# shiyao-li/NextBestPath

Measured on AMD Instinct MI355X. Metric: exploration steps/s (+ NBP maps/s) at 256x256, higher is better.
Workload: dtype f32

## Files before the change

nextbestpath_amd/csrc/nbp_conv.hip:

```cpp
#include "common.h"
#include "nbp_internal.h"
#include "nbp_first_conv.h"
#include <cstdlib>



template <int WM, int WN, int TM, int TN>
__global__ __launch_bounds__(256, 2) void igemm_conv_kernel(IgemmArgs a) {
    int zs = blockIdx.z;
    if (zs >= a.split_k) {
        zs -= a.split_k;
        a.src0 = a.g_src0; a.src1 = a.g_src1; a.wpk = a.g_wpk; a.scale = a.g_scale; a.shift = a.g_shift; a.out = a.g_out;
    }
    constexpr int BM = WM * TM * 32, BN = WN * TN * 32;
    constexpr int RA = BM / 32, RB = BN / 32;
    constexpr int STAGE = (BM + BN) * 32;
    static_assert(WM * WN == 4, "256-thread workgroup");
    extern __shared__ __attribute__((aligned(16))) float lds[];
    const int tid = threadIdx.x, lane = tid & 63, wave = tid >> 6;
    const int wm = wave / WN, wn = wave % WN;
    unsigned mt = blockIdx.x, nt = blockIdx.y;
    if (a.xcd_remap) {
        const unsigned L = blockIdx.x + gridDim.x * blockIdx.y, T = gridDim.x * gridDim.y;
        const unsigned xcd = L & 7u, idx = L >> 3, q = T >> 3, r = T & 7u;
// ... 638 lines not shown

__global__ __launch_bounds__(256) void conv_first_mfma_linear_kernel(const float* __restrict__ x, int B, int H, int W,
                                                                     const float* __restrict__ w, const float* __restrict__ scale,
                                                                     const float* __restrict__ shift, float* __restrict__ out) {
    auto st4 = [](float* p, const f32x4& v) { *reinterpret_cast<f32x4*>(p) = v; };
    conv_first_mfma_body<float, decltype(st4), false>(x, B, H, W, w, scale, shift, out, st4, nullptr);
}

static unsigned first_grid(long long M) {
    constexpr int cap = 512;
    const long long tiles = M / 256;
    return (unsigned)(tiles < cap ? tiles : cap);
}

int nbp_conv_first_amax_launch(const float* x_nchw, int B, int H, int W, const float* w_oihw, const float* scale, const float* shift,
                               float* out_nhwc, unsigned* amax_out, int* did_amax, hipStream_t st) {
    long long M = (long long)B * H * W;
    *did_amax = 0;
    if ((H & 7) == 0 && (W & 31) == 0) {
        conv_first_mfma_kernel<<<first_grid(M), 256, 0, st>>>(x_nchw, B, H, W, w_oihw, scale, shift, out_nhwc, amax_out);
        *did_amax = amax_out ? 1 : 0;
        return nbp_launch_status();
    }
    return nbp_conv_first_f32(x_nchw, B, H, W, w_oihw, scale, shift, out_nhwc, st);
}

extern "C" int nbp_conv_first_f32(const float* x_nchw, int B, int H, int W, const float* w_oihw, const float* scale,
                                  const float* shift, float* out_nhwc, void* stream) {
    NBP_ENTER();
    NBP_RETURN_IF(!x_nchw || !w_oihw || !scale || !shift || !out_nhwc, NBP_E_ARG);
    NBP_RETURN_IF(B < 1 || H < 1 || W < 1, NBP_E_ARG);
    long long M = (long long)B * H * W;
    if ((H & 7) == 0 && (W & 31) == 0) {
        conv_first_mfma_kernel<<<first_grid(M), 256, 0, (hipStream_t)stream>>>(x_nchw, B, H, W, w_oihw, scale, shift, out_nhwc, nullptr);
        return nbp_launch_status();
    }
    conv_first_kernel<<<(unsigned)nbp_cdiv(M, 64), 256, 0, (hipStream_t)stream>>>(x_nchw, B, H, W, w_oihw, scale,
                                                                                   shift, out_nhwc);
    return nbp_launch_status();
}

extern "C" int nbp_conv_first_linear_f32(const float* x_nchw, int B, int H, int W, const float* w_oihw, const float* scale,
                                         const float* shift, float* out_nhwc, void* stream) {
    NBP_ENTER();
    NBP_RETURN_IF(!x_nchw || !w_oihw || !scale || !shift || !out_nhwc || B < 1, NBP_E_ARG);
    NBP_RETURN_IF(H < 8 || W < 32 || (H & 7) || (W & 31), NBP_E_SHAPE);
    conv_first_mfma_linear_kernel<<<first_grid((long long)B * H * W), 256, 0, (hipStream_t)stream>>>(x_nchw, B, H, W, w_oihw, scale, shift, out_nhwc);
    return nbp_launch_status();
}

__global__ __launch_bounds__(256) void maxpool2_kernel(const float* __restrict__ in, int B, int H, int W, int C4,
                                                       float* __restrict__ out) {
    const int Ho = H >> 1, Wo = W >> 1;
    const long long total = (long long)B * Ho * Wo * C4;
    const f32x4* in4 = reinterpret_cast<const f32x4*>(in);
    f32x4* out4 = reinterpret_cast<f32x4*>(out);
    for (long long i = (long long)blockIdx.x * blockDim.x + threadIdx.x; i < total;
         i += (long long)gridDim.x * blockDim.x) {
        int c = (int)(i % C4);
        long long p = i / C4;
        int xo = (int)(p % Wo);
        long long q = p / Wo;
        int yo = (int)(q % Ho);
        int b = (int)(q / Ho);
        long long base = (((long long)b * H + 2 * yo) * W + 2 * xo) * C4 + c;
        f32x4 v0 = in4[base], v1 = in4[base + C4], v2 = in4[base + (long long)W * C4],
              v3 = in4[base + (long long)W * C4 + C4];
        f32x4 r;
#pragma unroll
        for (int e = 0; e < 4; ++e) r[e] = fmaxf(fmaxf(v0[e], v1[e]), fmaxf(v2[e], v3[e]));
        out4[i] = r;
    }
}

extern "C" int nbp_maxpool2_nhwc_f32(const float* in, int B, int H, int W, int C, float* out, void* stream) {
    NBP_ENTER();
    NBP_RETURN_IF(!in || !out, NBP_E_ARG);
    NBP_RETURN_IF(B < 1 || H < 2 || W < 2 || (H & 1) || (W & 1) || C < 4 || (C & 3), NBP_E_SHAPE);
    long long total = (long long)B * (H / 2) * (W / 2) * (C / 4);
    maxpool2_kernel<<<nbp_ew_grid(total, 256), 256, 0, (hipStream_t)stream>>>(in, B, H, W, C / 4, out);
    return nbp_launch_status();
}

__global__ __launch_bounds__(256) void psi_gate_kernel(const float* __restrict__ q, int F4,
                                                       const float* __restrict__ wpsi, const float* __restrict__ st,
                                                       const float* __restrict__ x, int C4, long long M,
                                                       float* __restrict__ out) {
    const int sub = threadIdx.x & 15;
    const f32x4* q4 = reinterpret_cast<const f32x4*>(q);
    const f32x4* w4 = reinterpret_cast<const f32x4*>(wpsi);
    const f32x4* x4 = reinterpret_cast<const f32x4*>(x);
    f32x4* o4 = reinterpret_cast<f32x4*>(out);
    const float s = st[0], t = st[1];
    const long long ppb = blockDim.x >> 4;
    for (long long m = (long long)blockIdx.x * ppb + (threadIdx.x >> 4); m < M; m += (long long)gridDim.x * ppb) {
        float acc = 0.f;
        for (int f = sub; f < F4; f += 16) {
            f32x4 a = q4[m * F4 + f], b = w4[f];
            acc = fmaf(a[0], b[0], acc); acc = fmaf(a[1], b[1], acc);
            acc = fmaf(a[2], b[2], acc); acc = fmaf(a[3], b[3], acc);
        }
        acc += __shfl_xor(acc, 8, 16);
        acc += __shfl_xor(acc, 4, 16);
        acc += __shfl_xor(acc, 2, 16);
        acc += __shfl_xor(acc, 1, 16);
        const float z = acc * s + t;
        const float psi = 1.f / (1.f + expf(-z));
        for (int c = sub; c < C4; c += 16) o4[m * C4 + c] = x4[m * C4 + c] * psi;
    }
}

extern "C" int nbp_psi_gate_f32(const float* q, int F, const float* w_psi, const float* s_t2, const float* x, int C,
                                long long M, float* out, void* stream) {
    NBP_ENTER();
    NBP_RETURN_IF(!q || !w_psi || !s_t2 || !x || !out, NBP_E_ARG);
    NBP_RETURN_IF(F < 4 || (F & 3) || C < 4 || (C & 3) || M < 1, NBP_E_SHAPE);
    psi_gate_kernel<<<nbp_ew_grid(M * 16, 256), 256, 0, (hipStream_t)stream>>>(q, F / 4, w_psi, s_t2, x, C / 4, M,
                                                                                out);
    return nbp_launch_status();
}

template <int NO>
__global__ __launch_bounds__(256) void final_1x1_kernel(const float* __restrict__ in, int B, int H, int W, int C4,
                                                        const float* __restrict__ w, const float* __restrict__ scale,
                                                        const float* __restrict__ shift, int sigmoid,
                                                        float* __restrict__ out) {
    const int sub = threadIdx.x & 15;
    const f32x4* in4 = reinterpret_cast<const f32x4*>(in);
    const f32x4* w4 = reinterpret_cast<const f32x4*>(w);
    const long long HW = (long long)H * W, M = (long long)B * HW;
    const long long ppb = blockDim.x >> 4;
    for (long long m = (long long)blockIdx.x * ppb + (threadIdx.x >> 4); m < M; m += (long long)gridDim.x * ppb) {
        float acc[NO];
#pragma unroll
        for (int o = 0; o < NO; ++o) acc[o] = 0.f;
        for (int c = sub; c < C4; c += 16) {
            f32x4 v = in4[m * C4 + c];
#pragma unroll
            for (int o = 0; o < NO; ++o) {
                f32x4 ww = w4[o * C4 + c];
                acc[o] = fmaf(v[0], ww[0], acc[o]); acc[o] = fmaf(v[1], ww[1], acc[o]);
                acc[o] = fmaf(v[2], ww[2], acc[o]); acc[o] = fmaf(v[3], ww[3], acc[o]);
            }
        }
#pragma unroll
        for (int o = 0; o < NO; ++o) {
            acc[o] += __shfl_xor(acc[o], 8, 16);
            acc[o] += __shfl_xor(acc[o], 4, 16);
            acc[o] += __shfl_xor(acc[o], 2, 16);
            acc[o] += __shfl_xor(acc[o], 1, 16);
        }
        if (sub == 0) {
            const long long b = m / HW, rem = m - b * HW;
#pragma unroll
            for (int o = 0; o < NO; ++o) {
                float v = acc[o] * scale[o] + shift[o];
                if (sigmoid) v = 1.f / (1.f + expf(-v));
                out[(b * NO + o) * HW + rem] = v;
            }
        }
    }
}

extern "C" int nbp_final_1x1_f32(const float* in, int B, int H, int W, int C, const float* w_oc, int n_out,
                                 const float* scale, const float* shift, int sigmoid, float* out_nchw, void* stream) {
    NBP_ENTER();
    NBP_RETURN_IF(!in || !w_oc || !scale || !shift || !out_nchw, NBP_E_ARG);
    NBP_RETURN_IF(B < 1 || H < 1 || W < 1 || C < 4 || (C & 3), NBP_E_SHAPE);
    long long M = (long long)B * H * W;
    int grid = nbp_ew_grid(M * 16, 256);
    hipStream_t st = (hipStream_t)stream;
    if (n_out == 8) final_1x1_kernel<8><<<grid, 256, 0, st>>>(in, B, H, W, C / 4, w_oc, scale, shift, sigmoid, out_nchw);
    else if (n_out == 1) final_1x1_kernel<1><<<grid, 256, 0, st>>>(in, B, H, W, C / 4, w_oc, scale, shift, sigmoid, out_nchw);
    else return NBP_E_SHAPE;
    return nbp_launch_status();
}

__global__ void nchw_to_nhwc_kernel(const float* __restrict__ in, int B, int C, long long HW, float* __restrict__ out) {
    const long long total = (long long)B * C * HW;
    for (long long i = (long long)blockIdx.x * blockDim.x + threadIdx.x; i < total;
         i += (long long)gridDim.x * blockDim.x) {
        int c = (int)(i % C);
        long long p = i / C;
        long long b = p / HW, hw = p - b * HW;
        out[i] = in[(b * C + c) * HW + hw];
    }
}
__global__ void nhwc_to_nchw_kernel(const float* __restrict__ in, int B, int C, long long HW, float* __restrict__ out) {
    const long long total = (long long)B * C * HW;
    for (long long i = (long long)blockIdx.x * blockDim.x + threadIdx.x; i < total;
         i += (long long)gridDim.x * blockDim.x) {
        long long hw = i % HW;
        long long p = i / HW;
        int c = (int)(p % C);
        long long b = p / C;
        out[i] = in[(b * HW + hw) * C + c];
    }
}
extern "C" int nbp_nchw_to_nhwc_f32(const float* in, int B, int C, int H, int W, float* out, void* stream) {
    NBP_ENTER();
    NBP_RETURN_IF(!in || !out || B < 1 || C < 1 || H < 1 || W < 1, NBP_E_ARG);
    long long total = (long long)B * C * H * W;
    nchw_to_nhwc_kernel<<<nbp_ew_grid(total, 256), 256, 0, (hipStream_t)stream>>>(in, B, C, (long long)H * W, out);
    return nbp_launch_status();
}
extern "C" int nbp_nhwc_to_nchw_f32(const float* in, int B, int C, int H, int W, float* out, void* stream) {
    NBP_ENTER();
    NBP_RETURN_IF(!in || !out || B < 1 || C < 1 || H < 1 || W < 1, NBP_E_ARG);
    long long total = (long long)B * C * H * W;
    nhwc_to_nchw_kernel<<<nbp_ew_grid(total, 256), 256, 0, (hipStream_t)stream>>>(in, B, C, (long long)H * W, out);
    return nbp_launch_status();
}
```

nextbestpath_amd/csrc/nbp_forward.hip:

```cpp
#include "common.h"
#include "nbp_internal.h"
#include <stdio.h>
#include <stdlib.h>
#include <string.h>

namespace {

enum Kind { K_FIRST, K_CONV3, K_ATT_G, K_ATT_X, K_PSI, K_FINAL };
struct LayerSpec { Kind kind; int cin, cout, k; };

struct Table {
    LayerSpec L[NBP_N_CONV];
    size_t w_off[NBP_N_CONV];
    size_t s_off[NBP_N_CONV], t_off[NBP_N_CONV];
    size_t total_floats;
    size_t w3_off[NBP_N_CONV];
    size_t w3u_off[NBP_N_CONV];
    bool is_up[NBP_N_CONV];
    int up_rank[NBP_N_CONV];
    size_t total3_bytes;
    size_t wup16_off[NBP_N_CONV], total_up16_bytes;
    size_t w1_off[NBP_N_CONV];
    int gate_rank[NBP_N_CONV];
    Table() {
// ... 201 lines not shown
                break;
        }
    }
    if (rc) { free(h); return rc; }
    *handle_out = h;
    return 0;
}

extern "C" int nbp_pack_weights(const void* const* w_host_array, const void* const* scale_host_array,
                                const void* const* shift_host_array, void* packed, size_t packed_bytes, void* stream,
                                nbp_weights** handle_out) {
    NBP_ENTER();
    return pack_weights_impl(w_host_array, scale_host_array, shift_host_array, packed, packed_bytes, stream, handle_out,
                             false);
}

extern "C" int nbp_pack_weights_bf16(const void* const* w_host_array, const void* const* scale_host_array,
                                     const void* const* shift_host_array, void* packed, size_t packed_bytes,
                                     void* stream, nbp_weights** handle_out) {
    NBP_ENTER();
    return pack_weights_impl(w_host_array, scale_host_array, shift_host_array, packed, packed_bytes, stream, handle_out,
                             true);
}

extern "C" size_t nbp_packed_weights_bytes_split(void) { return table().total_floats * sizeof(float) + table().total3_bytes; }
extern "C" int nbp_pack_weights_split(const void* const* w_host_array, const void* const* scale_host_array,
                                      const void* const* shift_host_array, void* packed, size_t packed_bytes,
                                      void* stream, nbp_weights** handle_out) {
    NBP_ENTER();
    return pack_weights_impl(w_host_array, scale_host_array, shift_host_array, packed, packed_bytes, stream, handle_out,
                             false, true);
}

extern "C" size_t nbp_packed_weights_bytes_bf16(void) { return table().total_floats * sizeof(float) + table().total_up16_bytes; }

extern "C" void nbp_free_weights(nbp_weights* handle) { free(handle); }

namespace {

struct Bump {
    char* base; size_t size, off; bool dry;
    template <typename T> T* take(size_t count) {
        size_t bytes = (count * sizeof(T) + 255) / 256 * 256;
        size_t o = off; off += bytes;
        if (dry) return (T*)(uintptr_t)256;
        return (T*)(base + o);
    }
};

struct Timer {
    hipStream_t st;
    nbp_layer_timing* out; int cap; int n;
    hipEvent_t ev[256];
    int nev;
    int begin() {
        nev = 0; n = 0;
        hipError_t e = hipEventCreate(&ev[0]);
        if (e != hipSuccess) return (int)e;
        nev = 1;
        return (int)hipEventRecord(ev[0], st);
    }
    void mark(const char* name, double flops, int tile, int split_k, long long M, int N, int K) {
        if (n >= cap || nev >= 256) return;
        if (hipEventCreate(&ev[nev]) != hipSuccess) return;
        (void)hipEventRecord(ev[nev], st);
        ++nev;
        nbp_layer_timing& t = out[n++];
        memset(&t, 0, sizeof(t));
        strncpy(t.name, name, sizeof(t.name) - 1);
        t.flops = flops; t.tile = tile; t.split_k = split_k; t.M = M; t.N = N; t.K = K;
    }
    int finish() {
        hipError_t e = hipStreamSynchronize(st);
        for (int i = 0; i + 1 < nev && i < n; ++i) {
            float ms = 0.f;
            (void)hipEventElapsedTime(&ms, ev[i], ev[i + 1]);
            out[i].ms = ms;
        }
        for (int i = 0; i < nev; ++i) (void)hipEventDestroy(ev[i]);
        return (int)e;
    }
};

struct NoCtx {
    int init(Bump&, hipStream_t, bool) { return 0; }
    void offer_gated(void*, void*) {}
    bool took_gated() { return false; }
    void offer_pool(void*) {}
    bool took_pool() { return false; }
    void offer_head(const float*, const float*, const float*, float*) {}
    bool took_head() { return false; }
};
struct PathF32 {
    typedef float T;
    typedef ConvOperands Ops;
    typedef NoCtx Ctx;
    static constexpr int CHUNK = 32;
    static ConvPlan plan(long long M, int N, int chunks, int groups, int H = 0, int ksize = 0, int ups = 0) {
        (void)ups;
        return nbp_plan_conv(M, N, chunks, 0, 0, groups, H, H, ksize);
    }
    static constexpr int MODE = 0;
    template <typename C>
    static int conv(C&, const nbp_weights*, const int*, const Ops& o, const Ops* o2, int C0, int C1, int ups, int B, int H, int ks,
                    int N, void* ws, size_t wsb, hipStream_t st) {
        return nbp_conv_igemm_launch_g(o, o2, C0, C1, ups, B, H, H, ks, N, 1, 0, 0, ws, wsb, st);
    }
    template <typename C>
    static int first(C&, const float* x, int B, int s, const nbp_weights* h, T* out, hipStream_t st) {
        return nbp_conv_first_f32(x, B, s, s, (const float*)h->w[0], h->scale[0], h->shift[0], out, st);
    }
    template <typename C>
    static int pool(C&, const T* in, int B, int H, int Cn, T* out, hipStream_t st) { return nbp_maxpool2_nhwc_f32(in, B, H, H, Cn, out, st); }
    template <typename C>
    static int gate(C&, const T* q, int F, const float* w, const float* s2, const T* x, int Cn, long long M, T* out, hipStream_t st) {
        return nbp_psi_gate_f32(q, F, w, s2, x, Cn, M, out, st);
    }
    static int head(const T* in, int B, int H, int C, const float* w, int no, const float* sc, const float* sh, int sig,
                    float* out, hipStream_t st) {
        return nbp_final_1x1_f32(in, B, H, H, C, w, no, sc, sh, sig, out, st);
    }
};
struct AmaxBook {
    unsigned* slots = nullptr;
    int next = 0, n = 0;
    hipStream_t st = nullptr;
    const void* key[128];
    unsigned* val[128];
    int init(Bump& bp, hipStream_t s, bool dry) {
        st = s; next = n = 0;
        slots = bp.take<unsigned>(128 * 64);
        return dry ? 0 : fill_f32(reinterpret_cast<float*>(slots), 0.f, 128 * 64, st);
    }
    unsigned* find(const void* p) const {
        for (int i = n - 1; i >= 0; --i) if (key[i] == p) return val[i];
        return nullptr;
    }
    void bind(const void* p, unsigned* v) { if (n < 128) { key[n] = p; val[n] = v; ++n; } }
    unsigned* unbound() { return next < 128 ? slots + 64 * next++ : nullptr; }
    unsigned* fresh(const void* p) { unsigned* v = next < 128 ? slots + 64 * next++ : nullptr; if (v) bind(p, v); return v; }
    void alias(const void* p, const void* of) { if (unsigned* v = find(of)) bind(p, v); }
    float* gated[2] = {nullptr, nullptr};
    bool gated_taken = false;
    void offer_gated(void* g0, void* g1) { gated[0] = (float*)g0; gated[1] = (float*)g1; gated_taken = false; }
    bool took_gated() { const bool t = gated_taken; gated[0] = gated[1] = nullptr; gated_taken = false; return t; }
    const float* psi_key[2] = {nullptr, nullptr};
    const float* psi_x[2] = {nullptr, nullptr};
    float* pool = nullptr;
    bool pool_taken = false;
    void offer_pool(void* p) { pool = (float*)p; pool_taken = false; }
    bool took_pool() { const bool t = pool_taken; pool = nullptr; pool_taken = false; return t; }
    ConvHead head = {nullptr, nullptr, nullptr, nullptr};
    bool head_taken = false;
    void offer_head(const float* w, const float* sc, const float* sh, float* out) { head = ConvHead{w, sc, sh, out}; head_taken = false; }
    bool took_head() { const bool t = head_taken; head = ConvHead{nullptr, nullptr, nullptr, nullptr}; head_taken = false; return t; }
    int ensure(const float* p, long long count, const unsigned** out) {
        unsigned* v = find(p);
        int rc = 0;
        if (!v) {
            v = fresh(p);
            if (!v) return NBP_E_WS;
            rc = nbp_amax_launch(p, count, v, st);
        }
        *out = v;
        return rc;
    }
};
struct PathSplit : PathF32 {
    typedef AmaxBook Ctx;
    static constexpr int MODE = 2;
    static ConvPlan plan(long long M, int N, int chunks, int groups, int H = 0, int ksize = 0, int ups = 0) {
        if (ksize == 1) return ConvPlan{NBP_TILE_SPLIT_GATE, 1, chunks};
        const ConvPlan p = nbp_plan_conv_split(M, N, chunks, 0, groups, H, H, ksize, ups);
        return p.tile ? p : PathF32::plan(M, N, chunks, groups, H, ksize);
    }
    static int conv(Ctx& ctx, const nbp_weights* h, const int* li, const Ops& o, const Ops* o2, int C0, int C1, int ups, int B,
                    int H, int ks, int N, void* ws, size_t wsb, hipStream_t st) {
        if (ks == 1 && C1 == C0 && C0 % 64 == 0 && !ups && h->w1[li[0]] && (!o2 || h->w1[li[1]])) {
            const long long M = (long long)B * H * H;
            ConvOperandsSplit s[2];
            for (int g = 0; g < (o2 ? 2 : 1); ++g) {
                const Ops& q = g ? *o2 : o;
                s[g] = ConvOperandsSplit{q.src0, q.src1, h->w1[li[g]], q.scale, q.shift, q.out, nullptr, nullptr, h->wamax1[li[g]], nullptr,
                                         nullptr, nullptr};
                int rc = ctx.ensure(q.src0, M * C0, &s[g].amax0);
                if (!rc) rc = ctx.ensure(q.src1, M * C1, &s[g].amax1);
                if (rc) return rc;
            }
            GatePsi psi;
            for (int g = 0; g < 2; ++g) {
                const int l = li[(g && o2) ? 1 : 0] + 2;
                psi.wpsi[g] = (const float*)h->w[l]; psi.st[g] = h->scale[l]; psi.gated[g] = ctx.gated[(g && o2) ? 1 : 0];
            }
            unsigned* gslot[2] = {nullptr, nullptr};
            if (ctx.gated[0]) for (int g = 0; g < (o2 ? 2 : 1); ++g) psi.gated_amax[g] = gslot[g] = ctx.unbound();
            static const int psi_on_load = nbp_tune_int("NBP_SPLIT_PSI_ON_LOAD", 1);
            const ConvPlan pc = nbp_plan_conv_split(M, C0, (C0 + C0) / 32 * 9, 0, o2 ? 2 : 1, H, H, 3, 0);
            psi.psi_only = psi_on_load && (C0 >= 128 || psi_on_load >= 2) && ctx.gated[0] && gslot[0] && (!o2 || gslot[1]) && pc.tile != 0 &&
                           M * C0 * 4 < (1ll << 31);
            int fused = 0;
            const int rc = nbp_gate1x1_split_launch_g(s[0], o2 ? &s[1] : nullptr, C0, M, N, 1, st, ctx.gated[0] ? &psi : nullptr, &fused);
            if (fused) {
                ctx.gated_taken = true;
                for (int g = 0; g < (o2 ? 2 : 1); ++g) {
                    if (gslot[g]) ctx.bind(ctx.gated[g], gslot[g]);
                    else ctx.alias(ctx.gated[g], (g ? *o2 : o).src1);
                    if (psi.psi_only) { ctx.psi_key[g] = ctx.gated[g]; ctx.psi_x[g] = (g ? *o2 : o).src1; }
                }
            }
            return rc;
        }
        const ConvPlan p = nbp_plan_conv_split((long long)B * H * H, N, (C0 + C1) / 32 * ks * ks, 0, o2 ? 2 : 1, H, H, ks, ups);
        if (!p.tile) return PathF32::conv(ctx, h, li, o, o2, C0, C1, ups, B, H, ks, N, ws, wsb, st);
        const long long hw = (long long)B * (ups ? H / 2 : H) * (ups ? H / 2 : H);
        ConvOperandsSplit s[2];
        for (int g = 0; g < (o2 ? 2 : 1); ++g) {
            const Ops& q = g ? *o2 : o;
            s[g] = ConvOperandsSplit{q.src0, q.src1, h->w3[li[g]], q.scale, q.shift, q.out, nullptr, nullptr, h->wamax[li[g]], nullptr,
                                     h->w3u[li[g]], h->wamax_u[li[g]]};
            int rc = ctx.ensure(q.src0, hw * C0, &s[g].amax0);
            if (!rc && C1) rc = ctx.ensure(q.src1, hw * C1, &s[g].amax1);
            if (rc) return rc;
            s[g].amax_out = ctx.fresh(q.out);
            for (int k = 0; k < 2; ++k)
                if (ctx.psi_key[k] && q.src0 == ctx.psi_key[k]) {
                    s[g].src0 = ctx.psi_x[k]; s[g].psi0 = ctx.psi_key[k];
                    ctx.psi_key[k] = nullptr; ctx.psi_x[k] = nullptr;
                }
        }
        float* pools[2] = {ctx.pool, nullptr};
        int pooled = 0, headed = 0;
        const int rc = nbp_conv_split_launch_g(s[0], o2 ? &s[1] : nullptr, C0, C1, ups, B, H, H, ks, N, 1, 0, ws, wsb, st,
                                               (ctx.pool && !o2) ? pools : nullptr, &pooled, (ctx.head.out && !o2) ? &ctx.head : nullptr,
                                               &headed);
        if (headed) ctx.head_taken = true;
        if (pooled) {
            ctx.pool_taken = true;
            ctx.alias(ctx.pool, o.out);
        }
        return rc;
    }
    static int first(Ctx& ctx, const float* x, int B, int s, const nbp_weights* h, T* out, hipStream_t st) {
        unsigned* slot = ctx.fresh(out);
        int did = 0;
        const int rc = nbp_conv_first_amax_launch(x, B, s, s, (const float*)h->w[0], h->scale[0], h->shift[0], out, slot, &did, st);
        if (!did && slot) --ctx.n;
        return rc;
    }
    static int pool(Ctx& ctx, const T* in, int B, int H, int Cn, T* out, hipStream_t st) {
        ctx.alias(out, in);
        return nbp_maxpool2_nhwc_f32(in, B, H, H, Cn, out, st);
    }
    static int gate(Ctx& ctx, const T* q, int F, const float* w, const float* s2, const T* x, int Cn, long long M, T* out,
                    hipStream_t st) {
        ctx.alias(out, x);
        return nbp_psi_gate_f32(q, F, w, s2, x, Cn, M, out, st);
    }
};
struct Bf16Ctx : NoCtx {
    bf16_t* gated[2] = {nullptr, nullptr};
    bool gated_taken = false;
    void offer_gated(void* g0, void* g1) { gated[0] = (bf16_t*)g0; gated[1] = (bf16_t*)g1; gated_taken = false; }
    bool took_gated() { const bool t = gated_taken; gated[0] = gated[1] = nullptr; gated_taken = false; return t; }
    bf16_t* pool = nullptr;
    bool pool_taken = false;
    void offer_pool(void* p) { pool = (bf16_t*)p; pool_taken = false; }
    bool took_pool() { const bool t = pool_taken; pool = nullptr; pool_taken = false; return t; }
    ConvHead head = {nullptr, nullptr, nullptr, nullptr};
    bool head_taken = false;
    void offer_head(const float* w, const float* sc, const float* sh, float* out) { head = ConvHead{w, sc, sh, out}; head_taken = false; }
    bool took_head() { const bool t = head_taken; head = ConvHead{nullptr, nullptr, nullptr, nullptr}; head_taken = false; return t; }
};
struct PathBF16 {
    typedef bf16_t T;
    typedef ConvOperandsH Ops;
    typedef Bf16Ctx Ctx;
    static constexpr int CHUNK = 64;
    static ConvPlan plan(long long M, int N, int chunks, int groups, int H = 0, int ksize = 0, int ups = 0) {
        return nbp_plan_conv_bf16(M, N, chunks, 0, 0, groups, H, H, ksize, ups);
    }
    static constexpr int MODE = 1;
    static int conv(Ctx& ctx, const nbp_weights* h, const int* li, const Ops& o, const Ops* o2, int C0, int C1, int ups, int B, int H,
                    int ks, int N, void* ws, size_t wsb, hipStream_t st) {
        Ops a = o, b = o2 ? *o2 : o;
        a.wpk_up = (const bf16_t*)h->wup16[li[0]];
        if (o2) b.wpk_up = (const bf16_t*)h->wup16[li[1]];
        bf16_t* pools[2] = {ctx.pool, nullptr};
        int pooled = 0, headed = 0, psi_fused = 0;
        GatePsiH psi{{nullptr, nullptr}, {nullptr, nullptr}, {nullptr, nullptr}};
        const bool gate = ks == 1 && C1 == C0 && ctx.gated[0] && (!o2 || ctx.gated[1]);
        if (gate)
            for (int g = 0; g < (o2 ? 2 : 1); ++g) {
                const int l = li[g] + 2;
                psi.wpsi[g] = (const float*)h->w[l]; psi.st[g] = h->scale[l]; psi.gated[g] = ctx.gated[g];
            }
        const int rc = nbp_conv_igemm_bf16_launch_g(a, o2 ? &b : nullptr, C0, C1, ups, B, H, H, ks, N, 1, 0, 0, ws, wsb, st,
                                                    (ctx.pool && !o2) ? pools : nullptr, &pooled,
                                                    (ctx.head.out && !o2) ? &ctx.head : nullptr, &headed, gate ? &psi : nullptr, &psi_fused);
        if (pooled) ctx.pool_taken = true;
        if (headed) ctx.head_taken = true;
        if (psi_fused) ctx.gated_taken = true;
        return rc;
    }
    static int first(Ctx&, const float* x, int B, int s, const nbp_weights* h, T* out, hipStream_t st) {
        return nbp_conv_first_bf16_launch(x, B, s, s, (const float*)h->w[0], h->scale[0], h->shift[0], out, st);
    }
    static int pool(Ctx&, const T* in, int B, int H, int C, T* out, hipStream_t st) { return nbp_maxpool2_bf16_launch(in, B, H, H, C, out, st); }
    static int gate(Ctx&, const T* q, int F, const float* w, const float* s2, const T* x, int C, long long M, T* out, hipStream_t st) {
        return nbp_psi_gate_bf16_launch(q, F, w, s2, x, C, M, out, st);
    }
    static int head(const T* in, int B, int H, int C, const float* w, int no, const float* sc, const float* sh, int sig,
                    float* out, hipStream_t st) {
        return nbp_final_1x1_bf16_launch(in, B, H, H, C, w, no, sc, sh, sig, out, st);
    }
};

template <typename P>
size_t splitk_scratch_floats(long long M, int N, int cin_total, int taps, int groups, int H, int ups = 0) {
    ConvPlan p = P::plan(M, N, cin_total / P::CHUNK * taps, groups, H, taps == 9 ? 3 : 1, ups);
    return p.split_k > 1 ? (size_t)groups * p.split_k * M * N : 0;
}

template <typename P>
int run_forward(const nbp_weights* h, const float* x, int B, int S, float* out1, float* out2, Bump& bp,
                hipStream_t st, Timer* tm = nullptr) {
    typedef typename P::T T;
    typedef typename P::Ops Ops;
    char nm[48];
    const bool dry = bp.dry;
    const int enc[5] = {64, 128, 256, 512, 1024};
    int rc = 0;
    size_t sk = 0;
    {
        int s = S;
        sk = 0;
        for (int e = 0; e < 5; ++e, s /= 2) {
            long long M = (long long)B * s * s;
            if (e > 0) sk = max(sk, splitk_scratch_floats<P>(M, enc[e], enc[e - 1], 9, 1, s));
            sk = max(sk, splitk_scratch_floats<P>(M, enc[e], enc[e], 9, 1, s));
            if (e < 4) {
                for (int g = 1; g <= 2; ++g) {
                    sk = max(sk, splitk_scratch_floats<P>(M, enc[e], enc[e + 1], 9, g, s));
                    sk = max(sk, splitk_scratch_floats<P>(M, enc[e], enc[e + 1], 9, g, s, 1));
                    sk = max(sk, splitk_scratch_floats<P>(M, enc[e], enc[e], 9, g, s));
                    sk = max(sk, splitk_scratch_floats<P>(M, enc[e], 2 * enc[e], 9, g, s));
                    sk = max(sk, splitk_scratch_floats<P>(M, enc[e] / 2, 2 * enc[e], 1, g, s));
                }
            }
        }
    }
    float* skws = bp.take<float>(sk ? sk : 64);
    const size_t skbytes = sk * sizeof(float);
    typename P::Ctx ctx;
    rc = ctx.init(bp, st, dry);

    auto conv2 = [&](const char* name, int ng, const int* li, const T* const* s0, int C0, const T* const* s1,
                     int C1, int ups, int Hh, int ksize, int N, T* const* out) {
        if (dry || rc) return;
        Ops o[2];
        for (int g = 0; g < ng; ++g)
            o[g] = Ops{s0[g], s1 ? s1[g] : nullptr, (const T*)h->w[li[g]], h->scale[li[g]], h->shift[li[g]], out[g]};
        rc = P::conv(ctx, h, li, o[0], ng == 2 ? &o[1] : nullptr, C0, C1, ups, B, Hh, ksize, N, skws, skbytes, st);
        if (tm && !rc) {
            const long long M = (long long)B * Hh * Hh;
            const int K = (C0 + C1) * ksize * ksize;
            ConvPlan p = P::plan(M, N, K / P::CHUNK, ng, Hh, ksize, ups);
            tm->mark(name, 2.0 * ng * M * N * K, p.tile, p.split_k, M, N, K);
        }
    };
    auto conv = [&](const char* name, int li, const T* s0, int C0, const T* s1, int C1, int ups, int Hh,
                    int ksize, int N, T* out) {
        const T* s0a[1] = {s0};
        const T* s1a[1] = {s1};
        T* oa[1] = {out};
        conv2(name, 1, &li, s0a, C0, s1 ? s1a : nullptr, C1, ups, Hh, ksize, N, oa);
    };
    auto stamp = [&](const char* name, double flops, long long M, int N, int K) {
        if (tm && !dry && !rc) tm->mark(name, flops, -1, 1, M, N, K);
    };

    T* skip[5];
    int li = 0;
    int s = S;
    const T* prev = nullptr;
    T* pooled_next = nullptr;
    bool pool_fused = false;
    for (int e = 0; e < 5; ++e) {
        const int co = enc[e];
        const size_t n = (size_t)B * s * s * co;
        T* a = bp.take<T>(n);
        T* b = bp.take<T>(n);
        if (e == 0) {
            if (!dry && !rc) rc = P::first(ctx, x, B, s, h, a, st);
            stamp("Conv1.conv.0(first)", 2.0 * B * s * s * 64 * 45, (long long)B * s * s, 64, 45);
        } else {
            T* pooled = pooled_next;
            if (!dry && !rc && !pool_fused) rc = P::pool(ctx, prev, B, 2 * s, enc[e - 1], pooled, st);
            snprintf(nm, sizeof nm, "Maxpool%d", e);
            stamp(nm, 0, (long long)B * s * s, enc[e - 1], 0);
            snprintf(nm, sizeof nm, "Conv%d.conv.0", e + 1);
            conv(nm, li, pooled, enc[e - 1], nullptr, 0, 0, s, 3, co, a);
        }
        snprintf(nm, sizeof nm, "Conv%d.conv.3", e + 1);
        if (e < 4) {
            pooled_next = bp.take<T>((size_t)B * (s / 2) * (s / 2) * co);
            ctx.offer_pool(pooled_next);
        }
        conv(nm, li + 1, a, co, nullptr, 0, 0, s, 3, co, b);
        pool_fused = ctx.took_pool();
        li += 2;
        skip[e] = b; prev = b;
        if (e < 4) s /= 2;
    }
    const int li_d1 = 10, li_d2 = 22;
    bool head2_fused = false;
    const T* cur[2] = {skip[4], skip[4]};
    for (int Lv = 5; Lv >= 2; --Lv) {
        const int ng = Lv >= 4 ? 2 : 1;
        const int g0 = Lv >= 4 ? 0 : 1;
        const int co = enc[Lv - 2], ci = enc[Lv - 1];
        const int sr = S >> (Lv - 2);
        const long long M = (long long)B * sr * sr;
        const T* xs = skip[Lv - 2];
        T *dd[2], *q[2], *ag[2], *u[2], *o[2];
        int lis[2];
        const T *src[2], *xsa[2] = {xs, xs};
        for (int g = 0; g < ng; ++g) {
            dd[g] = bp.take<T>((size_t)M * co); q[g] = bp.take<T>((size_t)M * (co / 2)); ag[g] = bp.take<T>((size_t)M * co);
            u[g] = bp.take<T>((size_t)M * co); o[g] = bp.take<T>((size_t)M * co);
            const int d = g0 + g;
            lis[g] = (d == 0 ? li_d1 : li_d2) + (5 - Lv) * 6;
            src[g] = cur[d];
        }
        const char* tag = ng == 2 ? "{1,2}" : "2";
        auto shifted = [&](int k, int* dst) { for (int g = 0; g < ng; ++g) dst[g] = lis[g] + k; };
        int l[2];
        snprintf(nm, sizeof nm, "Up%d_%s.up.1", Lv, tag);
        shifted(0, l); conv2(nm, ng, l, src, ci, nullptr, 0, 1, sr, 3, co, dd);
        snprintf(nm, sizeof nm, "Att%d_%s.W_g+W_x", Lv, tag);
        ctx.offer_gated(ag[0], ng == 2 ? ag[1] : nullptr);
        shifted(1, l); conv2(nm, ng, l, (const T* const*)dd, co, xsa, co, 0, sr, 1, co / 2, q);
        const bool psi_fused = ctx.took_gated();
        for (int g = 0; g < ng && !dry && !rc && !psi_fused; ++g)
            rc = P::gate(ctx, q[g], co / 2, (const float*)h->w[lis[g] + 3], h->scale[lis[g] + 3], xs, co, M, ag[g], st);
        snprintf(nm, sizeof nm, "Att%d_%s.psi*x", Lv, tag);
        stamp(nm, 2.0 * ng * M * (co / 2), M, 1, co / 2);
        snprintf(nm, sizeof nm, "Up_conv%d_%s.conv.0", Lv, tag);
        shifted(4, l); conv2(nm, ng, l, (const T* const*)ag, co, (const T* const*)dd, co, 0, sr, 3, co, u);
        snprintf(nm, sizeof nm, "Up_conv%d_%s.conv.3", Lv, tag);
        if (Lv == 2 && !dry) ctx.offer_head((const float*)h->w[47], h->scale[47], h->shift[47], out2);
        shifted(5, l); conv2(nm, ng, l, (const T* const*)u, co, nullptr, 0, 0, sr, 3, co, o);
        if (Lv == 2) head2_fused = ctx.took_head();
        for (int g = 0; g < ng; ++g) cur[g0 + g] = o[g];
        if (Lv == 4) {
            if (!dry && !rc)
                rc = P::head(cur[0], B, S / 4, 256, (const float*)h->w[46], 8, h->scale[46], h->shift[46], 0, out1, st);
            stamp("Final1", 2.0 * B * (S / 4) * (S / 4) * 8 * 256, (long long)B * (S / 4) * (S / 4), 8, 256);
        }
    }
    if (!dry && !rc && !head2_fused)
        rc = P::head(cur[1], B, S, 64, (const float*)h->w[47], 1, h->scale[47], h->shift[47], 1, out2, st);
    stamp("Final2", 2.0 * B * S * S * 64, (long long)B * S * S, 1, 64);
    return rc;
}

}

template <typename P>
static size_t workspace_bytes_impl(int B, int S) {
    if (B < 1 || S < 16 || S % 16) return 0;
    Bump bp{nullptr, 0, 0, true};
    run_forward<P>(nullptr, nullptr, B, S, nullptr, nullptr, bp, nullptr);
    return bp.off + 256;
}

template <typename P>
static int forward_impl(const nbp_weights* handle, const float* x, int B, int S, float* out1, float* out2, void* ws,
                        size_t ws_bytes, void* stream, nbp_layer_timing* timings_host, int max_entries,
                        int* n_entries_host) {
    NBP_RETURN_IF(!handle || !x || !out1 || !out2 || !ws, NBP_E_ARG);
    NBP_RETURN_IF(handle->bf16 != (P::MODE == 1 ? 1 : 0) || (P::MODE == 2 && !handle->split), NBP_E_ARG);
    NBP_RETURN_IF(B < 1, NBP_E_ARG);
    NBP_RETURN_IF(S < 16 || S % 16, NBP_E_SHAPE);
    NBP_RETURN_IF(ws_bytes < workspace_bytes_impl<P>(B, S), NBP_E_WS);
    uintptr_t p = ((uintptr_t)ws + 255) / 256 * 256;
    Bump bp{(char*)p, ws_bytes, 0, false};
    if (!timings_host) return run_forward<P>(handle, x, B, S, out1, out2, bp, (hipStream_t)stream);
    NBP_RETURN_IF(!n_entries_host || max_entries < 1, NBP_E_ARG);
    static Timer tm;
    tm.st = (hipStream_t)stream; tm.out = timings_host; tm.cap = max_entries;
    int rc = tm.begin();
    if (rc) return rc;
    rc = run_forward<P>(handle, x, B, S, out1, out2, bp, (hipStream_t)stream, &tm);
    int rc2 = tm.finish();
    *n_entries_host = tm.n;
    return rc ? rc : rc2;
}

extern "C" size_t nbp_forward_workspace_bytes(int B, int S) { return workspace_bytes_impl<PathF32>(B, S); }
extern "C" size_t nbp_forward_workspace_bytes_bf16(int B, int S) { return workspace_bytes_impl<PathBF16>(B, S); }

extern "C" int nbp_forward_f32(const nbp_weights* handle, const float* x, int B, int S, float* out1, float* out2,
                               void* ws, size_t ws_bytes, void* stream) {
    NBP_ENTER();
    return forward_impl<PathF32>(handle, x, B, S, out1, out2, ws, ws_bytes, stream, nullptr, 0, nullptr);
}

extern "C" size_t nbp_forward_workspace_bytes_split(int B, int S) { return workspace_bytes_impl<PathSplit>(B, S); }
extern "C" int nbp_forward_split_f32(const nbp_weights* handle, const float* x, int B, int S, float* out1, float* out2,
                                     void* ws, size_t ws_bytes, void* stream) {
    NBP_ENTER();
    return forward_impl<PathSplit>(handle, x, B, S, out1, out2, ws, ws_bytes, stream, nullptr, 0, nullptr);
}
extern "C" int nbp_forward_timed_split_f32(const nbp_weights* handle, const float* x, int B, int S, float* out1,
                                           float* out2, void* ws, size_t ws_bytes, void* stream,
                                           nbp_layer_timing* timings_host, int max_entries, int* n_entries_host) {
    NBP_ENTER();
    NBP_RETURN_IF(!timings_host || !n_entries_host, NBP_E_ARG);
    return forward_impl<PathSplit>(handle, x, B, S, out1, out2, ws, ws_bytes, stream, timings_host, max_entries,
                                   n_entries_host);
}

extern "C" int nbp_forward_bf16(const nbp_weights* handle, const float* x, int B, int S, float* out1, float* out2,
                                void* ws, size_t ws_bytes, void* stream) {
    NBP_ENTER();
    return forward_impl<PathBF16>(handle, x, B, S, out1, out2, ws, ws_bytes, stream, nullptr, 0, nullptr);
}
// ... 34 lines not shown
```

nextbestpath_amd/csrc/nbp_internal.h:

```cpp
#pragma once
#include "common.h"

typedef unsigned short bf16_t;

enum { NBP_TILE_AUTO = 0, NBP_TILE_128x128 = 1, NBP_TILE_256x64 = 2, NBP_TILE_256x32 = 3, NBP_TILE_128x64 = 4,
       NBP_TILE_64x128 = 5,
       NBP_TILE_HALO_128 = 6, NBP_TILE_HALO_64 = 7,
       NBP_TILE_HALO4_128 = 8, NBP_TILE_HALO4_64 = 9,
       NBP_TILE_SPLIT_HALO_64 = 10, NBP_TILE_SPLIT_UP = 11,
       NBP_TILE_HALO_UP_128 = 12, NBP_TILE_HALO_UP_64 = 13,
       NBP_TILE_RESERVED_14 = 14,
       NBP_TILE_SPLIT_HALO_R8 = 15, NBP_TILE_SPLIT_UP_R8 = 16,
       NBP_TILE_SPLIT_UP_DGRAD = 17,
       NBP_TILE_SPLIT_HALO_128 = 18,
       NBP_TILE_SPLIT_GATE = 19 };
struct TileInfo { int bm, bn; };
struct ConvPlan { int tile; int split_k; int chunks_per_split; int finish; };

struct IgemmArgs {
    const float* src0;
    const float* src1;
    int C0, C1;
    int cc0;
    int ups;
    int H, W;
    int Hs, Ws;
    int taps;
    const float* wpk;
    int N;
    const float* scale;
    const float* shift;
    int relu;
    float* out;
    long long M;
    int split_k;
    int chunks_total;
    int chunks_per_split;
    unsigned bytes0, bytes1;
    unsigned bytesw;
    float* partial;
    int groups;
    const float* g_src0;
    const float* g_src1;
    const float* g_wpk;
    const float* g_scale;
    const float* g_shift;
    float* g_out;
    int xcd_remap;
};
struct ConvOperands { const float* src0; const float* src1; const float* wpk; const float* scale; const float* shift; float* out; };
ConvPlan nbp_plan_conv(long long M, int N, int chunks_total, int tile, int split_k, int groups, int H = 0, int W = 0,
                       int ksize = 0);
int nbp_conv_igemm_launch_g(const ConvOperands& o, const ConvOperands* o2, int C0, int C1, int ups, int B, int H, int W,
                            int ksize, int N, int relu, int split_k, int tile, void* ws, size_t ws_bytes, hipStream_t st);

struct ConvOperandsSplit {
    const float* src0; const float* src1; const void* planes; const float* scale; const float* shift; float* out;
    const unsigned* amax0; const unsigned* amax1; const unsigned* wamax; unsigned* amax_out;
    const void* planes_up; const unsigned* wamax_up;
    const float* psi0 = nullptr;
};
ConvPlan nbp_plan_conv_split(long long M, int N, int chunks_total, int split_k, int groups, int H, int W, int ksize, int ups = 0);
int nbp_pack_upconv_weight_split_launch(const float* w_oihw, int N, int C, void* dst, unsigned* wamax_out, hipStream_t st, int one = 0);
struct ConvHead { const float* w; const float* scale; const float* shift; float* out; };
int nbp_conv_split_launch_g(const ConvOperandsSplit& o, const ConvOperandsSplit* o2, int C0, int C1, int ups, int B, int H, int W,
                            int ksize, int N, int relu, int split_k, void* ws, size_t ws_bytes, hipStream_t st,
                            float* const* pool_out = nullptr, int* pooled = nullptr, const struct ConvHead* head = nullptr,
                            int* headed = nullptr, double* bn_part = nullptr, int* bn_rows = nullptr, int one = 0);
int nbp_pack_conv_weight_split_launch(const float* w_oihw, int N, int C, int ksize, const float* scale_or_null, int c_off,
                                      int c_total, void* dst, unsigned* wamax_out, hipStream_t st, int one = 0);
int nbp_amax_launch(const float* x, long long n, unsigned* amax_inout, hipStream_t st);
int nbp_wgrad_split_launch(const float* src0, int C0, const float* src1, int C1, int ups, int B, int H, int W, const float* dy, int N,
                           int n_tiles, int splits, unsigned* amax3, const unsigned* amax0_in, const unsigned* amax1_in,
                           const unsigned* amaxy_in, float* part, hipStream_t st);
int nbp_pack_gate_weight_split_launch(const float* wg, const float* scale_g, const float* wx, const float* scale_x, int N, int C,
                                      void* dst, unsigned* wamax_out, hipStream_t st);
struct GatePsi { const float* wpsi[2]; const float* st[2]; float* gated[2]; unsigned* gated_amax[2] = {nullptr, nullptr};
                 int psi_only = 0; };
int nbp_gate1x1_split_launch_g(const ConvOperandsSplit& o, const ConvOperandsSplit* o2, int C, long long M, int N, int relu,
                               hipStream_t st, const GatePsi* psi = nullptr, int* fused = nullptr);
int nbp_conv_first_amax_launch(const float* x_nchw, int B, int H, int W, const float* w_oihw, const float* scale, const float* shift,
                               float* out_nhwc, unsigned* amax_out, int* did_amax, hipStream_t st);

struct ConvOperandsH { const bf16_t* src0; const bf16_t* src1; const bf16_t* wpk; const float* scale; const float* shift; bf16_t* out;
                       const bf16_t* wpk_up; };
ConvPlan nbp_plan_conv_bf16(long long M, int N, int chunks_total, int tile, int split_k, int groups, int H = 0, int W = 0,
                            int ksize = 0, int ups = 0);
int nbp_pack_upconv_weight_bf16_launch(const float* w_oihw, int N, int C, bf16_t* dst, hipStream_t st);
struct GatePsiH { const float* wpsi[2]; const float* st[2]; bf16_t* gated[2]; };
int nbp_conv_igemm_bf16_launch_g(const ConvOperandsH& o, const ConvOperandsH* o2, int C0, int C1, int ups, int B, int H,
                                 int W, int ksize, int N, int relu, int split_k, int tile, void* ws, size_t ws_bytes,
                                 hipStream_t st, bf16_t* const* pool_out = nullptr, int* pooled = nullptr,
                                 const struct ConvHead* head = nullptr, int* headed = nullptr, const GatePsiH* psi = nullptr,
                                 int* psi_fused = nullptr);
int nbp_conv_first_bf16_launch(const float* x_nchw, int B, int H, int W, const float* w_oihw, const float* scale,
                               const float* shift, bf16_t* out_nhwc, hipStream_t st);
int nbp_maxpool2_bf16_launch(const bf16_t* in, int B, int H, int W, int C, bf16_t* out, hipStream_t st);
int nbp_psi_gate_bf16_launch(const bf16_t* q, int F, const float* w_psi, const float* s_t2, const bf16_t* x, int C,
                             long long M, bf16_t* out, hipStream_t st);
int nbp_final_1x1_bf16_launch(const bf16_t* in, int B, int H, int W, int C, const float* w_oc, int n_out,
                              const float* scale, const float* shift, int sigmoid, float* out_nchw, hipStream_t st);

constexpr int NBP_FR_MAX_R = 31, NBP_FR_MAX_D = 8;
constexpr int NBP_FR_ROWS = 2 * NBP_FR_MAX_R + 1;
struct NbpSectorRows { unsigned char lo[8][NBP_FR_ROWS], hi[8][NBP_FR_ROWS]; };
bool nbp_sector_rows(int R, NbpSectorRows* out);
void nbp_unknown_words_launch(const float* maps6, int B, int S, int dilate, unsigned long long* seen, unsigned long long* occ,
                              unsigned long long* near_d, unsigned long long* unknown, hipStream_t st);
```

Before: 2414.

## Compute psi-only per pixel and apply gating on conv load; add row-batched final 1x1 head

In the split path, the attention gate no longer writes a full psi*x tensor. A new kernel computes one psi scalar per pixel for both groups in one launch and records psi/x aliases, so the following conv can apply the gate when it loads x. This removes a full read and write of the gated activation tensor, but it relies on the conv consumer honouring the psi keys. A second change adds a final 1x1 head kernel that keeps the weights in LDS and registers and processes several rows per thread, in place of the generic head for C=256 and 8 outputs.

```diff
diff --git a/nextbestpath_amd/csrc/nbp_conv.hip b/nextbestpath_amd/csrc/nbp_conv.hip
--- a/nextbestpath_amd/csrc/nbp_conv.hip
+++ b/nextbestpath_amd/csrc/nbp_conv.hip
@@ -744,6 +744,21 @@
     return nbp_launch_status();
 }
 
+__device__ __forceinline__ float psi_of_pixel(const f32x4* __restrict__ q4, const f32x4* __restrict__ w4, int F4, long long m, int sub,
+                                              float s, float t) {
+    float acc = 0.f;
+    for (int f = sub; f < F4; f += 16) {
+        f32x4 a = q4[m * F4 + f], b = w4[f];
+        acc = fmaf(a[0], b[0], acc); acc = fmaf(a[1], b[1], acc);
+        acc = fmaf(a[2], b[2], acc); acc = fmaf(a[3], b[3], acc);
+    }
+    acc += __shfl_xor(acc, 8, 16);
+    acc += __shfl_xor(acc, 4, 16);
+    acc += __shfl_xor(acc, 2, 16);
+    acc += __shfl_xor(acc, 1, 16);
+    const float z = acc * s + t;
+    return 1.f / (1.f + expf(-z));
+}
 __global__ __launch_bounds__(256) void psi_gate_kernel(const float* __restrict__ q, int F4,
                                                        const float* __restrict__ wpsi, const float* __restrict__ st,
                                                        const float* __restrict__ x, int C4, long long M,
@@ -756,20 +771,35 @@
     const float s = st[0], t = st[1];
     const long long ppb = blockDim.x >> 4;
     for (long long m = (long long)blockIdx.x * ppb + (threadIdx.x >> 4); m < M; m += (long long)gridDim.x * ppb) {
-        float acc = 0.f;
-        for (int f = sub; f < F4; f += 16) {
-            f32x4 a = q4[m * F4 + f], b = w4[f];
-            acc = fmaf(a[0], b[0], acc); acc = fmaf(a[1], b[1], acc);
-            acc = fmaf(a[2], b[2], acc); acc = fmaf(a[3], b[3], acc);
-        }
-        acc += __shfl_xor(acc, 8, 16);
-        acc += __shfl_xor(acc, 4, 16);
-        acc += __shfl_xor(acc, 2, 16);
-        acc += __shfl_xor(acc, 1, 16);
-        const float z = acc * s + t;
-        const float psi = 1.f / (1.f + expf(-z));
+        const float psi = psi_of_pixel(q4, w4, F4, m, sub, s, t);
         for (int c = sub; c < C4; c += 16) o4[m * C4 + c] = x4[m * C4 + c] * psi;
     }
+}
+struct PsiOnlyArgs { const float* q[2]; const float* wpsi[2]; const float* st[2]; float* psi[2]; };
+__global__ __launch_bounds__(256) void psi_only_kernel(PsiOnlyArgs a, int F4, long long M) {
+    const int sub = threadIdx.x & 15, g = blockIdx.y;
+    const f32x4* q4 = reinterpret_cast<const f32x4*>(a.q[g]);
+    const f32x4* w4 = reinterpret_cast<const f32x4*>(a.wpsi[g]);
+    float* __restrict__ out = a.psi[g];
+    const float s = a.st[g][0], t = a.st[g][1];
+    const long long ppb = blockDim.x >> 4;
+    for (long long m = (long long)blockIdx.x * ppb + (threadIdx.x >> 4); m < M; m += (long long)gridDim.x * ppb) {
+        const float psi = psi_of_pixel(q4, w4, F4, m, sub, s, t);
+        if (sub == 0) out[m] = psi;
+    }
+}
+int nbp_psi_only_launch(const float* const* q, int F, const float* const* w_psi, const float* const* s_t2, long long M, float* const* psi,
+                        int groups, hipStream_t st) {
+    NBP_RETURN_IF(groups < 1 || groups > 2 || !q || !w_psi || !s_t2 || !psi, NBP_E_ARG);
+    NBP_RETURN_IF(F < 4 || (F & 3) || M < 1, NBP_E_SHAPE);
+    PsiOnlyArgs a;
+    for (int g = 0; g < 2; ++g) {
+        const int gi = g < groups ? g : 0;
+        NBP_RETURN_IF(!q[gi] || !w_psi[gi] || !s_t2[gi] || !psi[gi], NBP_E_ARG);
+        a.q[g] = q[gi]; a.wpsi[g] = w_psi[gi]; a.st[g] = s_t2[gi]; a.psi[g] = psi[gi];
+    }
+    psi_only_kernel<<<dim3((unsigned)nbp_ew_grid(M * 16, 256), (unsigned)groups), 256, 0, st>>>(a, F / 4, M);
+    return nbp_launch_status();
 }
 
 extern "C" int nbp_psi_gate_f32(const float* q, int F, const float* w_psi, const float* s_t2, const float* x, int C,
@@ -838,6 +868,81 @@
     return nbp_launch_status();
 }
 
+template <int NO, int K, int R>
+__global__ __launch_bounds__(256) void final_1x1_rows_kernel(const float* __restrict__ in, long long M, long long HW,
+                                                             const float* __restrict__ w, const float* __restrict__ scale,
+                                                             const float* __restrict__ shift, int sigmoid, float* __restrict__ out) {
+    static_assert(NO <= 16, "one lane of a pixel's 16 per output");
+    constexpr int C4 = 16 * K;
+    __shared__ f32x4 wl[NO * C4];
+    const int sub = threadIdx.x & 15;
+    const f32x4* in4 = reinterpret_cast<const f32x4*>(in);
+    for (int i = threadIdx.x; i < NO * C4; i += 256) wl[i] = reinterpret_cast<const f32x4*>(w)[i];
+    __syncthreads();
+    f32x4 ww[NO][K];
+#pragma unroll
+    for (int o = 0; o < NO; ++o)
+#pragma unroll
+        for (int k = 0; k < K; ++k) ww[o][k] = wl[o * C4 + sub + 16 * k];
+    const float sc = sub < NO ? scale[sub] : 0.f, sh = sub < NO ? shift[sub] : 0.f;
+    const long long stride = (long long)gridDim.x * 16;
+    for (long long m0 = (long long)blockIdx.x * 16 + (threadIdx.x >> 4); m0 < M; m0 += R * stride) {
+        f32x4 v[R][K];
+#pragma unroll
+        for (int r = 0; r < R; ++r)
+#pragma unroll
+            for (int k = 0; k < K; ++k) {
+                const long long m = m0 + r * stride;
+                v[r][k] = m < M ? in4[m * C4 + sub + 16 * k] : f32x4{0.f, 0.f, 0.f, 0.f};
+            }
+        float acc[R][NO];
+#pragma unroll
+        for (int r = 0; r < R; ++r)
+#pragma unroll
+            for (int o = 0; o < NO; ++o) acc[r][o] = 0.f;
+#pragma unroll
+        for (int k = 0; k < K; ++k)
+#pragma unroll
+            for (int o = 0; o < NO; ++o)
+#pragma unroll
+                for (int r = 0; r < R; ++r) {
+                    acc[r][o] = fmaf(v[r][k][0], ww[o][k][0], acc[r][o]); acc[r][o] = fmaf(v[r][k][1], ww[o][k][1], acc[r][o]);
+                    acc[r][o] = fmaf(v[r][k][2], ww[o][k][2], acc[r][o]); acc[r][o] = fmaf(v[r][k][3], ww[o][k][3], acc[r][o]);
+                }
+#pragma unroll
+        for (int r = 0; r < R; ++r) {
+            const long long m = m0 + r * stride;
+            float mine = 0.f;
+#pragma unroll
+            for (int o = 0; o < NO; ++o) {
+                acc[r][o] += __shfl_xor(acc[r][o], 8, 16);
+                acc[r][o] += __shfl_xor(acc[r][o], 4, 16);
+                acc[r][o] += __shfl_xor(acc[r][o], 2, 16);
+                acc[r][o] += __shfl_xor(acc[r][o], 1, 16);
+                if (sub == o) mine = acc[r][o];
+            }
+            if (sub < NO && m < M) {
+                const long long b = m / HW, rem = m - b * HW;
+                float y = mine * sc + sh;
+                if (sigmoid) y = 1.f / (1.f + expf(-y));
+                out[(b * NO + sub) * HW + rem] = y;
+            }
+        }
+    }
+}
+
+int nbp_final_1x1_rows_launch(const float* in, int B, int H, int W, int C, const float* w_oc, int n_out, const float* scale,
+                              const float* shift, int sigmoid, float* out_nchw, hipStream_t st) {
+    static const int rows = nbp_tune_int("NBP_FINAL1_ROWS", 1);
+    if (!rows || C != 256 || n_out != 8) return nbp_final_1x1_f32(in, B, H, W, C, w_oc, n_out, scale, shift, sigmoid, out_nchw, st);
+    NBP_RETURN_IF(!in || !w_oc || !scale || !shift || !out_nchw, NBP_E_ARG);
+    NBP_RETURN_IF(B < 1 || H < 1 || W < 1, NBP_E_SHAPE);
+    const long long HW = (long long)H * W, M = (long long)B * HW;
+    const long long blocks = nbp_cdiv(M, 16);
+    final_1x1_rows_kernel<8, 4, 4><<<(unsigned)(blocks < 512 ? blocks : 512), 256, 0, st>>>(in, M, HW, w_oc, scale, shift, sigmoid, out_nchw);
+    return nbp_launch_status();
+}
+
 __global__ void nchw_to_nhwc_kernel(const float* __restrict__ in, int B, int C, long long HW, float* __restrict__ out) {
     const long long total = (long long)B * C * HW;
     for (long long i = (long long)blockIdx.x * blockDim.x + threadIdx.x; i < total;
diff --git a/nextbestpath_amd/csrc/nbp_forward.hip b/nextbestpath_amd/csrc/nbp_forward.hip
--- a/nextbestpath_amd/csrc/nbp_forward.hip
+++ b/nextbestpath_amd/csrc/nbp_forward.hip
@@ -307,6 +307,13 @@
     }
 };
 
+template <typename P>
+int gates_each(typename P::Ctx& ctx, int ng, typename P::T* const* q, int F, const float* const* w, const float* const* s2,
+               const typename P::T* x, int Cn, long long M, typename P::T* const* out, hipStream_t st) {
+    int rc = 0;
+    for (int g = 0; g < ng && !rc; ++g) rc = P::gate(ctx, q[g], F, w[g], s2[g], x, Cn, M, out[g], st);
+    return rc;
+}
 struct NoCtx {
     int init(Bump&, hipStream_t, bool) { return 0; }
     void offer_gated(void*, void*) {}
@@ -340,6 +347,10 @@
     template <typename C>
     static int gate(C&, const T* q, int F, const float* w, const float* s2, const T* x, int Cn, long long M, T* out, hipStream_t st) {
         return nbp_psi_gate_f32(q, F, w, s2, x, Cn, M, out, st);
+    }
+    static int gates(Ctx& ctx, int ng, T* const* q, int F, const float* const* w, const float* const* s2, const T* x, int Cn, long long M,
+                     int, T* const* out, hipStream_t st) {
+        return gates_each<PathF32>(ctx, ng, q, F, w, s2, x, Cn, M, out, st);
     }
     static int head(const T* in, int B, int H, int C, const float* w, int no, const float* sc, const float* sh, int sig,
                     float* out, hipStream_t st) {
@@ -481,6 +492,22 @@
         ctx.alias(out, x);
         return nbp_psi_gate_f32(q, F, w, s2, x, Cn, M, out, st);
     }
+    static int gates(Ctx& ctx, int ng, T* const* q, int F, const float* const* w, const float* const* s2, const T* x, int Cn, long long M,
+                     int H, T* const* out, hipStream_t st) {
+        static const int psi_on_load = nbp_tune_int("NBP_SPLIT_PSI_ON_LOAD", 1);
+        const bool psi_only = psi_on_load && (Cn >= 128 || psi_on_load >= 2) && M * Cn * 4 < (1ll << 31) &&
+                              nbp_plan_conv_split(M, Cn, (Cn + Cn) / 32 * 9, 0, ng, H, H, 3, 0).tile != 0;
+        if (!psi_only) return gates_each<PathSplit>(ctx, ng, q, F, w, s2, x, Cn, M, out, st);
+        for (int g = 0; g < ng; ++g) {
+            ctx.alias(out[g], x);
+            ctx.psi_key[g] = out[g]; ctx.psi_x[g] = x;
+        }
+        return nbp_psi_only_launch(q, F, w, s2, M, out, ng, st);
+    }
+    static int head(const T* in, int B, int H, int C, const float* w, int no, const float* sc, const float* sh, int sig,
+                    float* out, hipStream_t st) {
+        return nbp_final_1x1_rows_launch(in, B, H, H, C, w, no, sc, sh, sig, out, st);
+    }
 };
 struct Bf16Ctx : NoCtx {
     bf16_t* gated[2] = {nullptr, nullptr};
@@ -533,6 +560,10 @@
     static int pool(Ctx&, const T* in, int B, int H, int C, T* out, hipStream_t st) { return nbp_maxpool2_bf16_launch(in, B, H, H, C, out, st); }
     static int gate(Ctx&, const T* q, int F, const float* w, const float* s2, const T* x, int C, long long M, T* out, hipStream_t st) {
         return nbp_psi_gate_bf16_launch(q, F, w, s2, x, C, M, out, st);
+    }
+    static int gates(Ctx& ctx, int ng, T* const* q, int F, const float* const* w, const float* const* s2, const T* x, int C, long long M,
+                     int, T* const* out, hipStream_t st) {
+        return gates_each<PathBF16>(ctx, ng, q, F, w, s2, x, C, M, out, st);
     }
     static int head(const T* in, int B, int H, int C, const float* w, int no, const float* sc, const float* sh, int sig,
                     float* out, hipStream_t st) {
@@ -666,8 +697,11 @@
         ctx.offer_gated(ag[0], ng == 2 ? ag[1] : nullptr);
         shifted(1, l); conv2(nm, ng, l, (const T* const*)dd, co, xsa, co, 0, sr, 1, co / 2, q);
         const bool psi_fused = ctx.took_gated();
-        for (int g = 0; g < ng && !dry && !rc && !psi_fused; ++g)
-            rc = P::gate(ctx, q[g], co / 2, (const float*)h->w[lis[g] + 3], h->scale[lis[g] + 3], xs, co, M, ag[g], st);
+        if (!dry && !rc && !psi_fused) {
+            const float *wq[2], *sq[2];
+            for (int g = 0; g < ng; ++g) { wq[g] = (const float*)h->w[lis[g] + 3]; sq[g] = h->scale[lis[g] + 3]; }
+            rc = P::gates(ctx, ng, q, co / 2, wq, sq, xs, co, M, sr, ag, st);
+        }
         snprintf(nm, sizeof nm, "Att%d_%s.psi*x", Lv, tag);
         stamp(nm, 2.0 * ng * M * (co / 2), M, 1, co / 2);
         snprintf(nm, sizeof nm, "Up_conv%d_%s.conv.0", Lv, tag);
diff --git a/nextbestpath_amd/csrc/nbp_internal.h b/nextbestpath_amd/csrc/nbp_internal.h
--- a/nextbestpath_amd/csrc/nbp_internal.h
+++ b/nextbestpath_amd/csrc/nbp_internal.h
@@ -79,6 +79,10 @@
                  int psi_only = 0; };
 int nbp_gate1x1_split_launch_g(const ConvOperandsSplit& o, const ConvOperandsSplit* o2, int C, long long M, int N, int relu,
                                hipStream_t st, const GatePsi* psi = nullptr, int* fused = nullptr);
+int nbp_psi_only_launch(const float* const* q, int F, const float* const* w_psi, const float* const* s_t2, long long M, float* const* psi,
+                        int groups, hipStream_t st);
+int nbp_final_1x1_rows_launch(const float* in, int B, int H, int W, int C, const float* w_oc, int n_out, const float* scale,
+                              const float* shift, int sigmoid, float* out_nchw, hipStream_t st);
 int nbp_conv_first_amax_launch(const float* x_nchw, int B, int H, int W, const float* w_oihw, const float* scale, const float* shift,
                                float* out_nhwc, unsigned* amax_out, int* did_amax, hipStream_t st);
 
```

Measured after the change: 2413. About the same (-0.0%).
